# Aqasch/TensorRL-QAS

Hardware: AMD Instinct MI355X
Metric: VQE env-steps/sec (higher is better)
Workload: dtype f64

## Files before the change

tensorrl-qas_amd/csrc/vqe_device.h:

```cpp
#pragma once
#include <hip/hip_runtime.h>
#include <stdint.h>
#ifdef VQE_STAMPS
__device__ unsigned long long g_cby_dbg[8];
__device__ unsigned long long g_cby_in_out[2];
__device__ long long g_cby_t0_unused;
#if defined(__HIP_DEVICE_COMPILE__)
#define CBY_STAMP_RESET() long long cby_t0_ = (long long)__builtin_readcyclecounter(); (void)cby_t0_
#define CBY_STAMP(k)                                                                               \
  {                                                                                                \
    const long long t_ = (long long)__builtin_readcyclecounter();                                  \
    if (ctx.tid == 0 && Ctx::nth > 1) __hip_atomic_fetch_add(&g_cby_dbg[k], (unsigned long long)(t_ - cby_t0_), __ATOMIC_RELAXED, __HIP_MEMORY_SCOPE_AGENT); \
    cby_t0_ = (long long)__builtin_readcyclecounter();                                             \
  }
#else
#define CBY_STAMP_RESET()
#define CBY_STAMP(k)
#endif
#endif
#include "cobyla_m0.h"
#include "vqe_geo.h"

namespace vqe {

// ... 431 lines not shown
    const GateRec* g = staged ? gl : gsrc;
    uint32_t* xm = L.xm;
    uint32_t* zm = L.zm;
    for (int q = 0; q < n; ++q) { xm[q] = 1u << q; zm[q] = 1u << q; }
    uint32_t c = 0;
    int phase = 0, nops = 0;
    auto slot = [&](int q) {
      if (nops < A.max_ops) L.ops[nops] = Op{0u, zm[q], -1, OP_NOP};
      ++nops;
    };
    for (int i = 0; i < G; ++i) {
      if (i >= skip && i < skip_end) continue;
      const GateRec r = g[i];
      if (slots && (r.kind == G_DEPOL1 || r.kind == G_DEPOL2)) {
        slot(r.q0);
        if (r.kind == G_DEPOL2) slot(r.q1);
        continue;
      }
      switch (r.kind) {
        case G_CNOT:
          zm[r.q1] ^= zm[r.q0];
          xm[r.q0] ^= xm[r.q1];
          if ((c >> r.q0) & 1u) c ^= 1u << r.q1;
          break;
        case G_RX: case G_RY: case G_RZ:
          if (nops < A.max_ops)
            L.ops[nops] = Op{xm[r.q0], zm[r.q0], r.pidx, r.kind | (int)(((c >> r.q0) & 1u) << 8)};
          ++nops;
          break;
        case G_RXX: case G_RYY: case G_RZZ:
          if (nops < A.max_ops)
            L.ops[nops] = Op{xm[r.q0] ^ xm[r.q1], zm[r.q0] ^ zm[r.q1], r.pidx,
                             rot2_op(r.kind) | (int)((((c >> r.q0) ^ (c >> r.q1)) & 1u) << 8)};
          ++nops;
          break;
        default: break;
      }
    }
    int permuted = (c != 0);
    for (int q = 0; q < n; ++q) if (xm[q] != (1u << q)) permuted = 1;
    L.meta[0] = nops < A.max_ops ? nops : A.max_ops;
    L.meta[1] = (int32_t)c;
    L.meta[2] = phase;
    L.meta[3] = permuted;
    L.meta[6] = permuted;
    L.meta[7] = (int32_t)c;
  }
  __syncthreads();
}

template <int N>
__device__ __forceinline__ void patch_noise_wave(const BatchArgs& A, int b, uint64_t eval_id, const Lds& L, int skip,
                                                 bool canonical, int lane, int skip_end) {
  const int G = A.gate_count[b];
  const int4* gsrc = (const int4*)(A.gates + A.gate_begin[b]);
  {
    Op* exe = N >= 10 ? L.sched : L.ops;
    const int kmax = L.meta[0];
    const uint64_t lt_mask = lane ? (~0ull >> (64 - lane)) : 0ull;
    const uint64_t nkey = noise_key(A.noise.seed, (uint64_t)b, eval_id);
    uint32_t c = 0;
    int ny = 0, kbase = 0;
    int4 rnext = lane < G ? gsrc[lane] : make_int4(-1, 0, 0, 0);
    for (int base = 0; base < G; base += 64) {
      const int i = base + lane;
      int kind = -1, q0 = 0, q1 = 0, code = 0;
      const int4 r = rnext;
      if (i + 64 < G) rnext = gsrc[i + 64];
      if (i < G && !(i >= skip && i < skip_end)) {
        kind = r.x; q0 = r.y; q1 = r.z < 0 ? 0 : r.z;
        if (kind == G_DEPOL1 || kind == G_DEPOL2) {
          const double u = noise_uniform_k(nkey, (uint64_t)(i - ((skip >= 0 && i >= skip_end) ? skip_end - skip : 0)));
          if (kind == G_DEPOL1) { if (u < A.noise.p1) code = 1 + (int)(u / A.noise.p1 * 3.0); }
          else if (u < A.noise.p2) code = 1 + (int)(u / A.noise.p2 * 15.0);
        }
      }
      const int pa = kind == G_DEPOL1 ? code : (kind == G_DEPOL2 ? (code & 3) : 0);
      const int pb = kind == G_DEPOL2 ? (code >> 2) : 0;
      const uint32_t flip_a = (pa == 1 || pa == 2) ? 1u << q0 : 0u;
      const uint32_t flip_b = (pb == 1 || pb == 2) ? 1u << q1 : 0u;
      const uint32_t cnot_m = kind == G_CNOT ? 1u << q1 : 0u;
      const int nrec = ((kind >= G_RX && kind <= G_DEPOL1) || gate_is_rot2(kind)) ? 1 : (kind == G_DEPOL2 ? 2 : 0);
      const uint32_t w1 = flip_a | ((uint32_t)q0 << 16) | ((uint32_t)q1 << 24) | (gate_is_rot2(kind) ? 1u << 31 : 0u);
      const uint32_t w2 = cnot_m | (flip_b << 16);
      const uint64_t has1 = __ballot(nrec >= 1), has2 = __ballot(nrec == 2);
      const int k0 = kbase + __popcll(has1 & lt_mask) + __popcll(has2 & lt_mask);
      kbase += __popcll(has1) + __popcll(has2);
      ny += __popcll(__ballot(pa == 2)) + __popcll(__ballot(pb == 2));
      uint64_t inv0 = 0, inv1 = 0;
      const int cnt = G - base < 64 ? G - base : 64;
      int j0 = 0;
      if (c == 0) {
        const uint64_t flips = __ballot((flip_a | flip_b) != 0u);
        j0 = flips ? __ffsll((long long)flips) - 1 : cnt;
      }
      for (int j = j0; j < cnt; ++j) {
        const uint32_t a = (uint32_t)__builtin_amdgcn_readlane((int)w1, j);
        const uint32_t bw = (uint32_t)__builtin_amdgcn_readlane((int)w2, j);
        c ^= a & 0xffffu;
        const uint32_t b0 = ((c >> ((a >> 16) & 31u)) ^ ((c >> ((a >> 24) & 31u)) & (a >> 31))) & 1u;
        c ^= (0u - b0) & (bw & 0xffffu);
        inv0 |= (uint64_t)b0 << j;
        c ^= bw >> 16;
        inv1 |= (uint64_t)((c >> ((a >> 24) & 31u)) & 1u) << j;
      }
      auto apply = [&](int pk, int sign, int pauli) {
        if (pk < kmax) {
          Op* o = exe + L.sidx[pk];
          int kd = o->kind;
          if (pauli >= 0) kd = (kd & ~0xff) | ((pauli == 2 || pauli == 3) ? OP_PZ : OP_NOP);
          o->kind = (kd & ~0x100) | (sign << 8);
        }
      };
      if (nrec >= 1) apply(k0, (int)((inv0 >> lane) & 1ull), gate_is_rot(kind) ? -1 : pa);
      if (nrec == 2) apply(k0 + 1, (int)((inv1 >> lane) & 1ull), pb);
    }
    {
      const int ns = N >= 10 ? L.meta[4] : kmax;
      int lead = 0;
      for (int base = ((ns - 1) / 64) * 64; base >= 0; base -= 64) {
        const int k = base + lane;
        const int kd = k < ns ? exe[k].kind : 0;
        const bool nop = k < ns && (kd & 0xff) == OP_NOP;
        const uint64_t m = __ballot(nop);
        const uint64_t behind = lane < 63 ? (m >> (lane + 1)) : 0ull;
        const int in_chunk = 63 - lane;
        int run = behind == ~0ull >> (lane + 1) && lane < 63 ? in_chunk : (lane < 63 ? __ffsll((long long)~behind) - 1 : 0);
        if (run >= in_chunk) run = in_chunk + lead;
        if (k < ns) exe[k].kind = (kd & 0x00ffffff) | ((run < 255 ? run : 255) << 24);
        lead = (m == ~0ull) ? 64 + lead : __ffsll((long long)~m) - 1;
      }
    }
    if (lane == 0) {
      uint32_t cs = c;
      if (N >= 10 && canonical) {
        cs = 0;
        for (int q = 0; q < N; ++q) cs |= (uint32_t)parity32(A.ham.mrow[q] & c) << q;
      }
      L.meta[1] = (int32_t)cs;
      L.meta[2] = (3 * ny) & 3;
      L.meta[3] = L.meta[6] | (c != 0);
      L.meta[7] = (int32_t)c;
    }
  }
}

template <int N>
__device__ __forceinline__ void patch_noise(const BatchArgs& A, int b, uint64_t eval_id, const Lds& L, int skip,
                                            bool canonical, int skip_end = 0) {
  if (threadIdx.x < 64) patch_noise_wave<N>(A, b, eval_id, L, skip, canonical, (int)threadIdx.x, skip_end);
  __syncthreads();
}

}
#include "vqe_reg.h"
namespace vqe {

template <int N>
__device__ __forceinline__ void compile_all(const BatchArgs& A, int b, uint64_t eval_id, const Lds& L, int skip = -1,
                                            bool canonical = true, bool slots = false, int skip_end = 0) {
  compile_ops(A, b, eval_id, L, skip, slots, skip_end);
  if constexpr (N < 10) {
    if (slots) {
      for (int k = threadIdx.x; k < L.meta[0]; k += (int)blockDim.x) L.sidx[k] = (uint16_t)k;
      __syncthreads();
    }
  }
  if constexpr (N >= kRegMinQubits) {
    if (threadIdx.x == 0) schedule_ops<N>(L);
    __syncthreads();
    if (canonical) {
      uint32_t zrow = 0, cbit = 0;
      if (threadIdx.x < N) {
        const uint32_t m = A.ham.mrow[threadIdx.x];
        for (int q = 0; q < N; ++q) if ((m >> q) & 1u) zrow ^= L.zm[q];
        cbit = (uint32_t)parity32(m & (uint32_t)L.meta[1]) << threadIdx.x;
      }
      uint32_t cnew = cbit;
#pragma unroll
      for (int o = 8; o > 0; o >>= 1) cnew |= __shfl_xor(cnew, o, 16);
      __syncthreads();
      if (threadIdx.x < N) L.zm[threadIdx.x] = zrow;
      if (threadIdx.x == 0) L.meta[1] = (int32_t)cnew;
      __syncthreads();
    }
  }
}

template <int N, bool SLOTS = true>
__device__ __forceinline__ void run_ops(const Lds& L, const double* theta, int P, int p_hole = -1) {
  constexpr int kThreads = Geo<N>::NT;
  constexpr uint32_t DIM = 1u << N;
  constexpr int NP = (DIM / 2 + kThreads - 1) / kThreads;
  constexpr int NA = (DIM + kThreads - 1) / kThreads;
  const int tid = threadIdx.x;
  for (int j = tid; j < P; j += kThreads) {
    if (j == p_hole) continue;
    double s, c;
    sincos(0.5 * theta[j - (p_hole >= 0 && j > p_hole)], &s, &c);
    L.cs[j] = make_double2(c, s);
  }
  __syncthreads();
  const int nops = L.meta[0];
  for (int o = 0; o < nops; ++o) {
    const Op op = L.ops[o];
    const int kind = op.kind & 0xff;
    if constexpr (SLOTS) o += (int)((uint32_t)op.kind >> 24);
    if (kind == OP_NOP) continue;
    const int inv = (op.kind >> 8) & 1;
    if (op_is_pair(kind)) {
      const double2 cs = L.cs[op.pidx];
      const int hb = 31 - __clz((int)op.xm);
      if (kind == OP_RX) {
#pragma unroll
        for (int k = 0; k < NP; ++k) {
          const uint32_t q = tid + k * kThreads;
          if (DIM / 2 >= kThreads || q < DIM / 2) {
            const uint32_t p0 = insert0(q, hb), p1 = p0 ^ op.xm;
            const double2 a0 = L.psi[p0], a1 = L.psi[p1];
            L.psi[p0] = make_double2(cs.x * a0.x - cs.y * a1.y, cs.x * a0.y + cs.y * a1.x);
            L.psi[p1] = make_double2(cs.x * a1.x - cs.y * a0.y, cs.x * a1.y + cs.y * a0.x);
          }
        }
      } else if (kind == OP_RY) {
#pragma unroll
        for (int k = 0; k < NP; ++k) {
          const uint32_t q = tid + k * kThreads;
          if (DIM / 2 >= kThreads || q < DIM / 2) {
            const uint32_t p0 = insert0(q, hb), p1 = p0 ^ op.xm;
            const double s0 = (parity32(p0 & op.zm) ^ inv) ? -cs.y : cs.y;
            const double2 a0 = L.psi[p0], a1 = L.psi[p1];
            L.psi[p0] = make_double2(cs.x * a0.x + s0 * a1.x, cs.x * a0.y + s0 * a1.y);
            L.psi[p1] = make_double2(cs.x * a1.x - s0 * a0.x, cs.x * a1.y - s0 * a0.y);
          }
        }
      } else {
#pragma unroll
        for (int k = 0; k < NP; ++k) {
          const uint32_t q = tid + k * kThreads;
          if (DIM / 2 >= kThreads || q < DIM / 2) {
            const uint32_t p0 = insert0(q, hb), p1 = p0 ^ op.xm;
            const double s0 = (parity32(p0 & op.zm) ^ inv) ? cs.y : -cs.y;
            const double2 a0 = L.psi[p0], a1 = L.psi[p1];
            L.psi[p0] = make_double2(cs.x * a0.x - s0 * a1.y, cs.x * a0.y + s0 * a1.x);
            L.psi[p1] = make_double2(cs.x * a1.x - s0 * a0.y, cs.x * a1.y + s0 * a0.x);
          }
        }
      }
    } else if (kind == OP_RZ) {
      const double2 cs = L.cs[op.pidx];
#pragma unroll
      for (int k = 0; k < NA; ++k) {
        const uint32_t p = tid + k * kThreads;
        if (DIM >= kThreads || p < DIM) {
          const double s = (parity32(p & op.zm) ^ inv) ? -cs.y : cs.y;
          const double2 a = L.psi[p];
          L.psi[p] = make_double2(cs.x * a.x - s * a.y, cs.x * a.y + s * a.x);
        }
      }
    } else if (kind == OP_PZ) {
#pragma unroll
      for (int k = 0; k < NA; ++k) {
        const uint32_t p = tid + k * kThreads;
        if ((DIM >= kThreads || p < DIM) && (parity32(p & op.zm) ^ inv)) {
          const double2 a = L.psi[p];
          L.psi[p] = make_double2(-a.x, -a.y);
        }
      }
    }
    __syncthreads();
  }
  if (L.meta[3]) {
    const uint32_t c = (uint32_t)L.meta[1];
    double2 tmp[NA];
#pragma unroll
    for (int k = 0; k < NA; ++k) {
      const uint32_t i = tid + k * kThreads;
      if (DIM >= kThreads || i < DIM) {
        uint32_t v = i ^ c, p = 0;
#pragma unroll
        for (int q = 0; q < N; ++q) p ^= ((v >> q) & 1u) ? L.xm[q] : 0u;
        tmp[k] = L.psi[p];
      }
    }
    __syncthreads();
#pragma unroll
    for (int k = 0; k < NA; ++k) {
      const uint32_t i = tid + k * kThreads;
      if (DIM >= kThreads || i < DIM) L.psi[i] = tmp[k];
    }
    __syncthreads();
  }
}

template <int N>
__device__ __forceinline__ void load_init(const Lds& L, const double2* init) {
  constexpr int kThreads = Geo<N>::NT;
  constexpr uint32_t DIM = 1u << N;
  constexpr int NA = (DIM + kThreads - 1) / kThreads;
#pragma unroll
  for (int k = 0; k < NA; ++k) {
    const uint32_t p = threadIdx.x + k * kThreads;
    if (DIM >= kThreads || p < DIM) L.psi[p] = init[p];
  }
}


constexpr int kEnergyBatch = 4;

#define VQE_ENERGY_PAIRS(X, HB, DEXPR)                                                             \
  {                                                                                                \
    const uint32_t base = insert0(tid, (HB)) << 4, basex = base ^ ((X) << 4);                     \
    uint32_t kbit[KB > 0 ? KB : 1];                                                                \
    _Pragma("unroll") for (int i = 0; i < KB; ++i)                                                \
      kbit[i] = 16u << (LT + i + ((LT + i) >= (HB) ? 1 : 0));                                     \
    double p0s = 0.0, p1s = 0.0;                                                                   \
    _Pragma("unroll") for (int k0 = 0; k0 < NP; k0 += kEnergyBatch) {                             \
      constexpr int NB = NP < kEnergyBatch ? NP : kEnergyBatch;                                   \
      double2 pa[NB], pb[NB];                                                                      \
      _Pragma("unroll") for (int kk = 0; kk < NB; ++kk) {                                         \
        const int k = k0 + kk;                                                                     \
        uint32_t kc = 0;                                                                           \
        _Pragma("unroll") for (int i = 0; i < KB; ++i) if ((k >> i) & 1) kc ^= kbit[i];           \
        const bool live = FULL || tid + (uint32_t)k * kThreads < DIM / 2;                         \
        pb[kk] = live ? *(const double2*)(psi_b + (base ^ kc)) : make_double2(0.0, 0.0);         \
        pa[kk] = live ? *(const double2*)(psi_b + (basex ^ kc)) : make_double2(0.0, 0.0);        \
      }                                                                                            \
      __builtin_amdgcn_sched_barrier(0);                                                           \
      _Pragma("unroll") for (int kk = 0; kk < NB; ++kk) {                                         \
        const int k = k0 + kk;                                                                     \
        const double v = (pa[kk].x * pb[kk].x + pa[kk].y * pb[kk].y) * (DEXPR);                   \
        if (k & 1) p1s += v; else p0s += v;                                                       \
      }                                                                                            \
    }                                                                                              \
    acc0 += p0s;                                                         \
    acc1 += p1s;                                                                                   \
  }

#define VQE_ENERGY_CONSUME(G, D)                                                                   \
  {                                                                                                \
    const GroupMeta m = L.gm[G];                                                                   \
    const uint32_t x = (uint32_t)__builtin_amdgcn_readfirstlane((int)m.x);                        \
    const int hb = __builtin_amdgcn_readfirstlane(m.hb);                                          \
    VQE_ENERGY_PAIRS(x, hb, D[k])                                                                  \
  }

template <int N>
__device__ __forceinline__ void energy_real_lds(const Lds& L, const double* __restrict__ tables, int g0, int g1,
                                                double& acc0, double& acc1) {
  constexpr int kThreads = Geo<N>::NT;
  constexpr uint32_t DIM = 1u << N;
  constexpr int NP = (DIM / 2 + kThreads - 1) / kThreads;
  constexpr int LT = Geo<N>::LT;
  constexpr int KB = N > LT + 1 ? N - LT - 1 : 0;
// ... 308 lines not shown
    for (int j = 0; j < PD - 1; ++j) {
#pragma unroll
      for (int k = 0; k < NP / 2; ++k) buf[j][k] = buf_load_d2(rt, voff[k], (uint32_t)j * GSTRIDE);
      __builtin_amdgcn_sched_barrier(0);
    }
#pragma unroll
    for (int k = 0; k < NP / 2; ++k) buf[PD - 1][k] = make_double2(0.0, 0.0);
    double2 bA[HP], bB[HP];
    uint2 mh[2];
    uint4 mo[2][2];
    const uint32_t tid16 = stid << 4;
    uint32_t tb;
    int ccls;
#define VQE_R_FETCH(S, GI)                                                                         \
    {                                                                                              \
      const ClsMeta* cm_ = L.cm + ((GI) < ncls ? (GI) : ncls - 1);                                 \
      mh[S] = *(const uint2*)cm_;                                                                  \
      mo[S][0] = *(const uint4*)cm_->off;                                                          \
      if constexpr (NP > 4) mo[S][1] = *(const uint4*)(cm_->off + 4);                             \
    }
#define VQE_R_OFF(S, J) ((J) == 0 ? mo[S][0].x : (J) == 1 ? mo[S][0].y : (J) == 2 ? mo[S][0].z : (J) == 3 ? mo[S][0].w : \
                         (J) == 4 ? mo[S][1].x : (J) == 5 ? mo[S][1].y : (J) == 6 ? mo[S][1].z : mo[S][1].w)
#define VQE_R_LOAD(S, HH, PB)                                                                      \
    _Pragma("unroll") for (int kk = 0; kk < HP; ++kk)                                             \
      PB[kk] = lds_load_d2(psi_l, tb + VQE_R_OFF(S, (HH) * HP + kk));
#define VQE_R_OWN(C, J) own[(((J) >> (C)) << ((C) + 1)) | ((J) & ((1 << (C)) - 1))]
#define VQE_R_DV(D, J) (((J) & 1) ? D[(J) / 2].y : D[(J) / 2].x)
#define VQE_R_COMP_C(C, HH, PB, D)                                                                 \
    if constexpr (HP == 4)                                                                         \
      pair_fma4(acc0, acc1, VQE_R_OWN(C, (HH) * 4), VQE_R_OWN(C, (HH) * 4 + 1), VQE_R_OWN(C, (HH) * 4 + 2),     \
                VQE_R_OWN(C, (HH) * 4 + 3), PB, VQE_R_DV(D, (HH) * 4), VQE_R_DV(D, (HH) * 4 + 1),            \
                VQE_R_DV(D, (HH) * 4 + 2), VQE_R_DV(D, (HH) * 4 + 3));                                       \
    else if constexpr (HP == 2)                                                                    \
      pair_fma2(acc0, acc1, VQE_R_OWN(C, (HH) * 2), VQE_R_OWN(C, (HH) * 2 + 1), PB, VQE_R_DV(D, (HH) * 2),     \
                VQE_R_DV(D, (HH) * 2 + 1));                                                                  \
    else                                                                                           \
      pair_fma1(acc0, VQE_R_OWN(C, (HH)), PB, VQE_R_DV(D, (HH)));
#define VQE_R_BODY(C, JJ)                                                                          \
    {                                                                                              \
      VQE_R_COMP_C(C, 0, bA, buf[JJ])                                                              \
      __builtin_amdgcn_sched_barrier(0);                                                           \
      tb = tid16 ^ mh[((JJ) + 1) & 1].x;                                                           \
      VQE_R_LOAD(((JJ) + 1) & 1, 0, bA)                                                            \
      __builtin_amdgcn_sched_barrier(0);                                                           \
      VQE_R_COMP_C(C, 1, bB, buf[JJ])                                                              \
    }
    VQE_R_FETCH(0, 0)
    VQE_R_FETCH(1, 1)
    tb = tid16 ^ mh[0].x;
    VQE_R_LOAD(0, 0, bA)
    for (int g = 0; g < ncls; g += PD) {
#pragma unroll
      for (int j = 0; j < PD; ++j) {
        {
          const int sl = (j + PD - 1) % PD;
          int gr = (j == 0) ? (g == 0 ? PD - 1 : g - 1 + PD) : g + j - 1 + PD;
          gr = gr < ncls ? gr : ncls - 1;
          const uint32_t soff = (uint32_t)gr * GSTRIDE;
#pragma unroll
          for (int k = 0; k < NP / 2; ++k) buf[sl][k] = buf_load_d2(rt, voff[k], soff);
        }
        ccls = __builtin_amdgcn_readfirstlane((int)mh[j & 1].y);
        VQE_R_LOAD(j & 1, 1, bB)
        VQE_R_FETCH(j & 1, g + j + 2)
        __builtin_amdgcn_sched_barrier(0);
        switch (ccls) {
          case 0: VQE_R_BODY(0, j) break;
          case 1: VQE_R_BODY(1, j) break;
          case 2: if constexpr (R > 2) VQE_R_BODY(2, j) break;
          default: if constexpr (R > 3) VQE_R_BODY(3, j) break;
        }
        __builtin_amdgcn_sched_barrier(0);
      }
    }
#undef VQE_R_FETCH
#undef VQE_R_OFF
#undef VQE_R_LOAD
#undef VQE_R_OWN
#undef VQE_R_DV
#undef VQE_R_COMP_C
#undef VQE_R_BODY
  }
  after_pairs();
  unit_energy<N>(L, H, acc0, acc1);
  const int g1 = g0 + H.n_real;
  energy_real_lds<N>(L, tables, gc, g1, acc0, acc1);
  energy_imag_lds<N>(L, tables, g1, H.n_groups, acc0);
  return block_sum<Geo<N>::NW>(acc0 + acc1, L.red);
}

template <int N, bool SLOTS = false, class Hook = NoHook>
__device__ __forceinline__ double lds_evaluate(const BatchArgs& A, const Lds& L, const double* theta, int P,
                                               int p_hole = -1, Hook after_pairs = Hook(), bool cs_ready = false) {
#ifdef VQE_STAMPS
  const long long t0 = clock64();
#endif
  if constexpr (N >= kRegMinQubits) {
    run_ops_reg<N, SLOTS>(L, A.init, theta, P, p_hole, A.dbg, cs_ready);
  } else {
    load_init<N>(L, A.init);
    __syncthreads();
    run_ops<N, SLOTS>(L, theta, P, p_hole);
  }
#ifdef VQE_STAMPS
  const long long t1 = clock64();
#endif
  double e;
  if constexpr (N >= kRegMinQubits) e = reg_energy<N>(L, A.ham, after_pairs); else e = lds_energy<N>(L, A.ham);
#ifdef VQE_STAMPS
  if (threadIdx.x == 0) {
    atomicAdd(A.dbg + 0, 1ull);
    atomicAdd(A.dbg + 1, (unsigned long long)(t1 - t0));
    atomicAdd(A.dbg + 2, (unsigned long long)(clock64() - t1));
  }
#endif
  return e;
}

struct NoSide { __device__ __forceinline__ void operator()() const {} };

template <int K>
struct KeepRegs {
  double2 v;
  KeepRegs<K - 1> rest;
  template <class F> __device__ __forceinline__ void load(F f, int k = 0) { v = f(k); rest.load(f, k + 1); }
  template <class F> __device__ __forceinline__ void store(F f, int k = 0) const { f(k, v); rest.store(f, k + 1); }
};
template <>
struct KeepRegs<0> {
  template <class F> __device__ __forceinline__ void load(F, int = 0) {}
  template <class F> __device__ __forceinline__ void store(F, int = 0) const {}
};

template <int N, bool WIDE = (N >= 10 && Geo<N>::NT >= 256)>
struct StagedCobyla {
  static constexpr int kThreads = Geo<N>::NT;
  typedef cby::CobylaM0<WaveCtx, false, lds_double> CobL;
  static constexpr bool kBlock = WIDE && Geo<N>::NT >= 256;
  static constexpr bool kRowsG = WIDE && Geo<N>::NT == 64;
  typedef cby::CobylaM0<WaveCtx, false, double> CobG;
  typedef cby::CobylaM0<WaveRowsCtx, false, double> CobR;
  __device__ __forceinline__ bool rows_ctx() const { return kRowsG && n > 32; }
#ifndef VQE_BLOCK_TILE
#define VQE_BLOCK_TILE 1
#endif
  static constexpr bool kBlockTile = VQE_BLOCK_TILE && ((size_t)16 << N) >= (Geo<N>::NT / 64) * kCobTileBytes + 4096;
  typedef cby::CobylaM0<BlockCtx<Geo<N>::NT, kBlockTile>, false, double> CobB;
  double* red;
  bool block;
  double* gmem;
  double* lmem;
  double* tile;
  int* pub;
  int n, words;
  bool staged;
  bool resident;
  int want, nfvals;
#ifndef VQE_STAGE_PREFETCH
#define VQE_STAGE_PREFETCH 1
#endif
#ifndef VQE_LIGHT_OUT
#define VQE_LIGHT_OUT 0
#endif
  static constexpr bool PRE = VQE_STAGE_PREFETCH && N >= 10 && Geo<N>::NT >= 256;
  KeepRegs<PRE ? 6 : 0> pre;
  bool pre_valid;
  __device__ __forceinline__ void init(double* global_scratch, const Lds& L, int n_) {
    pre_valid = false;
    gmem = global_scratch;
    resident = L.cob != nullptr;
    lmem = resident ? L.cob : (double*)L.psi;
    tile = L.tile;
    pub = (int*)(L.red + 8);
    n = n_;
    words = (int)cby::scratch_doubles(n, WaveCtx::kPad);
    red = L.red;
    block = kBlock && n > 64;
    staged = resident || (!block && (size_t)words * 8 <= ((size_t)16 << N));
    if (block) words = (int)cby::scratch_doubles(n, CobB::P);
    if (!staged && !block) {
      const int pad = rows_ctx() ? CobR::P : CobG::P;
      words = (int)cby::scratch_doubles_ld(n, pad, cby::lead_dim_global(cby::padded(n, pad)));
    }
  }
  __device__ __forceinline__ double* x() const { return resident ? lmem : gmem; }
  __device__ __forceinline__ const double* state() const { return (resident ? lmem : gmem) + words - cby::kStateDoubles; }
  static constexpr int kStage = 6;
  __device__ __forceinline__ void prefetch() {
    if constexpr (PRE) {
      if (!staged || resident) return;
      const double2* s = (const double2*)gmem;
      const int nw = (words + 1) / 2;
      pre.load([&](int k) {
        const int i = (int)threadIdx.x + k * kThreads;
        return s[i < nw ? i : nw - 1];
      });
      pre_valid = true;
    }
  }
  __device__ __forceinline__ void in() {
    if (!staged || resident) return;
    const double2* s = (const double2*)gmem;
    double2* d = (double2*)lmem;
    const int nw = (words + 1) / 2;
    int first = threadIdx.x;
    if constexpr (PRE) {
      if (pre_valid) {
        pre.store([&](int k, const double2& v) {
          const int i = (int)threadIdx.x + k * kThreads;
          if (i < nw) d[i] = v;
        });
        pre_valid = false;
        first += kStage * kThreads;
      }
    }
    for (int i0 = first; i0 < nw; i0 += kStage * kThreads) {
      double2 v[kStage];
#pragma unroll
      for (int k = 0; k < kStage; ++k) {
        const int i = i0 + k * kThreads;
        v[k] = s[i < nw ? i : nw - 1];
      }
#pragma unroll
      for (int k = 0; k < kStage; ++k) asm volatile("" : "+v"(v[k].x), "+v"(v[k].y));
#pragma unroll
      for (int k = 0; k < kStage; ++k) {
        const int i = i0 + k * kThreads;
        if (i < nw) d[i] = v[k];
      }
    }
    __syncthreads();
  }
  __device__ __forceinline__ bool out(bool full = true, double2* cs_out = nullptr, int P = 0, int p_hole = -1) {
    if (threadIdx.x == 0) { pub[0] = want; pub[1] = nfvals; }
    __syncthreads();
    want = pub[0]; nfvals = pub[1];
    if (!staged || resident) return false;
    const bool light = VQE_LIGHT_OUT && !full && want && cs_out != nullptr;
    if (light) {
      for (int j = threadIdx.x; j < P; j += kThreads) {
        if (j == p_hole) continue;
        double sn, cn;
        sincos(0.5 * lmem[j - (p_hole >= 0 && j > p_hole)], &sn, &cn);
        cs_out[j] = make_double2(cn, sn);
      }
    }
    const double2* s = (const double2*)lmem;
    double2* d = (double2*)gmem;
    const int nw = (words + 1) / 2;
    for (int i0 = threadIdx.x; i0 < nw; i0 += kStage * kThreads) {
      double2 v[kStage];
#pragma unroll
      for (int k = 0; k < kStage; ++k) {
        const int i = i0 + k * kThreads;
        v[k] = s[i < nw ? i : nw - 1];
      }
#pragma unroll
      for (int k = 0; k < kStage; ++k) asm volatile("" : "+v"(v[k].x), "+v"(v[k].y));
#pragma unroll
      for (int k = 0; k < kStage; ++k) {
        const int i = i0 + k * kThreads;
        if (i < nw) d[i] = v[k];
      }
    }
    if (light) {
      asm volatile("s_waitcnt lgkmcnt(0)\n\ts_barrier" ::: "memory");
      return true;
    }
    __syncthreads();
    return false;
  }
  template <bool FIRST, class Cob, class Ptr>
  __device__ __forceinline__ void call(Ptr mem, double f, double rhobeg, double rhoend, int maxfun) {
    Cob cob;
    cob.ctx.tid = Cob::P == 0 ? 0 : (int)(threadIdx.x % (unsigned)decltype(cob.ctx)::nth);
    if constexpr (!std::is_base_of<WaveCtx, decltype(cob.ctx)>::value) cob.ctx.red = red;
    if constexpr (decltype(cob.ctx)::kTile) {
      if constexpr (std::is_base_of<WaveCtx, decltype(cob.ctx)>::value) {
        cob.ctx.tile = (lds_double*)tile;
        cob.ctx.shared = (lds_double*)tile + Cob::kTileDoubles;
      } else {
        cob.ctx.tile = (lds_double*)lmem + (threadIdx.x >> 6) * Cob::kTileDoubles;
        cob.ctx.shared = (lds_double*)lmem + (kThreads / 64) * Cob::kTileDoubles;
      }
    }
    int nn = n;
    if constexpr (N >= 10) asm volatile("" : "+s"(mem), "+s"(nn));
    cob.bind(mem, nn);
    if (FIRST) {
      want = cob.start(rhobeg, rhoend, maxfun);
    } else {
      cob.load_state();
      want = cob.tell(f);
    }
    nfvals = cob.nfvals;
    cob.save_state();
  }
  bool cs_ready;
  template <bool FIRST, class Side>
  __device__ __forceinline__ int run(double f, double rhobeg, double rhoend, int maxfun, Side side, bool full = true,
                                     double2* cs_out = nullptr, int P = 0, int p_hole = -1) {
#ifdef VQE_STAMPS
    const long long t0 = clock64();
#endif
    in();
#ifdef VQE_STAMPS
    const long long t1 = clock64();
#endif
    if (kBlock && block) {
      if constexpr (kBlock) {
        if (kThreads == 64 || (threadIdx.x >= 64 && threadIdx.x < 128)) side();
        call<FIRST, CobB>(gmem, f, rhobeg, rhoend, maxfun);
      }
    } else if (threadIdx.x < 64) {
      if (staged) call<FIRST, CobL>((lds_double*)lmem, f, rhobeg, rhoend, maxfun);
      else if (rows_ctx()) {
        if constexpr (kRowsG) call<FIRST, CobR>(gmem, f, rhobeg, rhoend, maxfun);
      } else call<FIRST, CobG>(gmem, f, rhobeg, rhoend, maxfun);
      if constexpr (kThreads == 64) side();
    } else if (threadIdx.x < 128) {
#ifdef VQE_STAMPS
      const long long ts0 = clock64();
#endif
      side();
#ifdef VQE_STAMPS
      if (threadIdx.x == 64 && !FIRST) atomicAdd(&g_cby_dbg[6], (unsigned long long)(clock64() - ts0));
#endif
    }
#ifdef VQE_STAMPS
    const long long t2 = clock64();
#endif
    cs_ready = out(full, cs_out, P, p_hole);
#ifdef VQE_STAMPS
    if (threadIdx.x == 0 && !FIRST) {
      atomicAdd(&g_cby_dbg[7], (unsigned long long)(t2 - t1));
      atomicAdd(&g_cby_in_out[0], (unsigned long long)(t1 - t0));
      atomicAdd(&g_cby_in_out[1], (unsigned long long)(clock64() - t2));
    }
#endif
    return want;
  }
  __device__ __forceinline__ int start(double rhobeg, double rhoend, int maxfun, bool full = true, double2* cs_out = nullptr,
                                       int P = 0, int p_hole = -1) {
    return run<true>(0.0, rhobeg, rhoend, maxfun, NoSide(), full, cs_out, P, p_hole);
  }
  template <class Side>
  __device__ __forceinline__ int tell(double f, unsigned long long* __restrict__ dbg, Side side, bool full = true,
                                      double2* cs_out = nullptr, int P = 0, int p_hole = -1) {
#ifdef VQE_STAMPS
    const long long t0 = clock64();
#endif
    const int w = run<false>(f, 0.0, 0.0, 0, side, full, cs_out, P, p_hole);
#ifdef VQE_STAMPS
    if (threadIdx.x == 0) atomicAdd(dbg + 4, (unsigned long long)(clock64() - t0));
#endif
    return w;
  }
};

template <int N>
__global__ void __launch_bounds__(Geo<N>::NT) k_lds_energy(BatchArgs A) {
  extern __shared__ __attribute__((aligned(16))) unsigned char smem[];
  const Lds L = carve(smem, N, A.max_ops, A.max_params, A.ham.n_groups, A.max_pair);
  const int b = blockIdx.x;
  const bool noisy = (A.noise.p1 > 0.0 || A.noise.p2 > 0.0);
  stage_groups(A.ham, L);
  if constexpr (N >= 10) stage_cls<N>(A.ham, L);
  compile_all<N>(A, b, 0, L, -1, true, noisy);
  if (noisy) patch_noise<N>(A, b, A.noise.eval_base, L, -1, true);
  double e = lds_evaluate<N, true>(A, L, A.theta + A.par_begin[b], A.par_count[b]);
  if (A.noise.shot_sigma != 0.0) e += A.noise.shot_sigma * noise_gauss(A.noise.seed, (uint64_t)b, A.noise.eval_base);
  if (threadIdx.x == 0) { A.fout[b] = e; if (A.nfev) A.nfev[b] = 1; }
}

template <int N>
__global__ void __launch_bounds__(Geo<N>::NT) k_lds_state(BatchArgs A) {
  constexpr int kThreads = Geo<N>::NT;
  extern __shared__ __attribute__((aligned(16))) unsigned char smem[];
  const Lds L = carve(smem, N, A.max_ops, A.max_params, A.ham.n_groups, A.max_pair);
  const bool noisy_state = (A.noise.p1 > 0.0 || A.noise.p2 > 0.0);
  compile_all<N>(A, 0, 0, L, -1, false, noisy_state);
  if (noisy_state) patch_noise<N>(A, 0, A.noise.eval_base, L, -1, false);
  if constexpr (N >= kRegMinQubits) {
    run_ops_reg<N, true>(L, A.init, A.theta + A.par_begin[0], A.par_count[0]);
  } else {
    load_init<N>(L, A.init);
    __syncthreads();
    run_ops<N>(L, A.theta + A.par_begin[0], A.par_count[0]);
  }
  const int ph = L.meta[2];
  for (uint32_t p = threadIdx.x; p < (1u << N); p += kThreads) {
    double2 a = L.psi[p];
    if (ph == 1) a = make_double2(-a.y, a.x);
    else if (ph == 2) a = make_double2(-a.x, -a.y);
    else if (ph == 3) a = make_double2(a.y, -a.x);
    A.state_out[p] = a;
  }
}

template <int N, bool WIDE = (N >= 10 && Geo<N>::NT >= 256), bool NOISY = false>
__global__ void __launch_bounds__(Geo<N>::NT, Geo<N>::WPS) k_lds_minimize(BatchArgs A) {
  constexpr int kThreads = Geo<N>::NT;
  extern __shared__ __attribute__((aligned(16))) unsigned char smem[];
  const Lds L = carve(smem, N, A.max_ops, A.max_params, A.ham.n_groups, A.max_pair);
  const int b = A.order[blockIdx.x];
  const int P = A.par_count[b];
  const double* theta = A.theta + A.par_begin[b];
  double* xout = A.xout + A.par_begin[b];
  constexpr bool noisy = NOISY;
  const int skip = A.new_gate ? A.new_gate[b] : -1;
  int p_hole = -1;
  int skip_end = skip + 1;
  if (skip >= 0) {
    const GateRec r = A.gates[A.gate_begin[b] + skip];
    if (gate_is_rot(r.kind)) p_hole = r.pidx;
    if (skip + 1 < A.gate_count[b]) {
      const GateRec f = A.gates[A.gate_begin[b] + skip + 1];
      if ((f.kind == G_DEPOL1 && r.kind >= G_RX && r.kind <= G_RZ && f.q0 == r.q0) ||
          (f.kind == G_DEPOL2 && r.kind == G_CNOT && f.q0 == r.q0 && f.q1 == r.q1))
        skip_end = skip + 2;
    }
  }
  const int Popt = P - (p_hole >= 0);
  stage_groups(A.ham, L);
  if constexpr (N >= 10) stage_cls<N>(A.ham, L);
  StagedCobyla<N, WIDE> sc;
  sc.cs_ready = false;
  const bool full_out = N < 10 || A.trace != nullptr;
  int phase = 0, nfev = 1;
  bool need_compile = true;
  bool patched = false;
  double fret = 0.0, flast = 0.0;
  if (Popt > 0) {
    sc.init(A.scratch + A.scratch_begin[b], L, Popt);
    for (int j = threadIdx.x; j < P; j += kThreads)
      if (j != p_hole) sc.x()[j - (p_hole >= 0 && j > p_hole)] = theta[j];
    __syncthreads();
    sc.start(A.rhobeg, A.rhoend, A.maxfun, full_out, L.cs, P, p_hole);
    phase = 1;
  }
  for (;;) {
    const double* th = phase == 0 ? theta : (phase == 1 ? sc.x() : xout);
    const int sk = phase == 2 ? -1 : skip;
    const int ske = phase == 2 ? 0 : skip_end;
    const int ph = phase == 2 ? -1 : p_hole;
    const uint64_t eid = A.noise.eval_base +
                         (phase == 1 ? (uint64_t)sc.nfvals : (phase == 2 ? (uint64_t)A.maxfun + 1 : 0));
    if (need_compile) { compile_all<N>(A, b, 0, L, sk, true, noisy, ske); need_compile = false; patched = false; }
    if (noisy && !patched) patch_noise<N>(A, b, eid, L, sk, true, ske);
    patched = false;
    const bool csr = phase == 1 && sc.cs_ready;
    double e = lds_evaluate<N, NOISY>(A, L, th, P, ph, [&]() { if (phase == 1) sc.prefetch(); }, csr);
    if (A.noise.shot_sigma != 0.0) e += A.noise.shot_sigma * noise_gauss(A.noise.seed, (uint64_t)b, eid);
    bool finished_opt = false;
    if (phase == 0) {
      fret = e;
      for (int j = threadIdx.x; j < P; j += kThreads) {
        xout[j] = A.env_step ? (double)(float)theta[j] : theta[j];
        A.xraw[A.par_begin[b] + j] = theta[j];
      }
      finished_opt = true;
    } else if (phase == 1) {
      flast = e;
      if (A.trace) {
        double* tr = A.trace + ((size_t)b * A.maxfun + (size_t)(sc.nfvals - 1)) * (size_t)(1 + A.max_params);
        if (threadIdx.x == 0) tr[0] = e;
        for (int j = threadIdx.x; j < Popt; j += kThreads) tr[1 + j] = sc.x()[j];
      }
#ifdef VQE_STAMPS
      const long long tt0 = clock64();
#endif
      const uint64_t eid_next = A.noise.eval_base + (uint64_t)sc.nfvals + 1;
      const int want = sc.tell(e, A.dbg, [&]() {
        if (noisy) patch_noise_wave<N>(A, b, eid_next, L, sk, true, (int)(threadIdx.x & 63), ske);
      }, full_out, L.cs, P, p_hole);
      patched = noisy && want;
#ifdef VQE_STAMPS
      if (threadIdx.x == 0) atomicAdd(A.dbg + 3, (unsigned long long)(clock64() - tt0));
#endif
      if (!want) {
        for (int j = threadIdx.x; j < P; j += kThreads) {
          const double v = (j == p_hole) ? theta[j] : sc.x()[j - (p_hole >= 0 && j > p_hole)];
          xout[j] = A.env_step ? (double)(float)v : v;
          A.xraw[A.par_begin[b] + j] = v;
        }
        const double* st = sc.state();
        fret = ((int)st[11] == cby::DONE_RHOEND && (int)st[10] == 1) ? flast : st[4];
        nfev = sc.nfvals;
        finished_opt = true;
      }
    } else {
      fret = e;
      break;
    }
    if (finished_opt) {
      if (!A.env_step) break;
      __syncthreads();
      phase = 2;
      need_compile = true;
    }
  }
  if (threadIdx.x == 0) { A.fout[b] = fret; A.nfev[b] = nfev; }
}

}
```

tensorrl-qas_amd/csrc/vqe_reg.h:

```cpp
#pragma once
#include "vqe_geo.h"

namespace vqe {

enum : int { OP_RELAYOUT = 5 };

struct LayoutRec {
  uint32_t e[5];
  uint32_t pos;
  uint32_t pos8;
  uint32_t pad;
};

struct Basis {
  uint32_t* e;
  int32_t* piv;
  int k;
  __device__ void clear() { k = 0; }
  __device__ uint32_t reduce(uint32_t v) const {
    for (int i = 0; i < k; ++i) if ((v >> piv[i]) & 1u) v ^= e[i];
    return v;
  }
  __device__ bool add(uint32_t v) {
    v = reduce(v);
// ... 34 lines not shown
  for (int i = 0; i < R; ++i) if ((svec >> i) & 1u) w ^= pat[i];
  return w;
}

template <int N>
__device__ __forceinline__ void schedule_ops(const Lds& L) {
  constexpr int R = N - Geo<N>::LT;
  const int nraw = L.meta[0];
  int ns = 0, nl = 0;
  Basis B;
  B.e = (uint32_t*)L.sb;
  B.piv = (int32_t*)L.sb + 8;
  auto open_layout = [&](int from) {
    B.clear();
    for (int k = from; k < nraw && B.k < R; ++k) {
      const int kd = L.ops[k].kind & 0xff;
      if (op_is_pair(kd)) B.add(L.ops[k].xm);
    }
    for (int b = N - 1; b >= 0 && B.k < R; --b) B.add(1u << b);
    emit_layout<N>(B, &L.lay[nl]);
    ++nl;
  };
  open_layout(0);
  for (int o = 0; o < nraw; ++o) {
    const Op op = L.ops[o];
    const int kd = op.kind & 0xff;
    uint32_t j = 0;
    if (op_is_pair(kd)) {
      if (B.reduce(op.xm) != 0) {
        open_layout(o);
        L.sched[ns++] = Op{(uint32_t)(nl - 1), 0u, -1, OP_RELAYOUT};
      }
      j = B.coords(op.xm);
    }
    uint32_t svec = 0;
    for (int i = 0; i < R; ++i) svec |= (uint32_t)parity32(op.zm & B.e[i]) << i;
    L.sidx[o] = (uint16_t)ns;
    L.sched[ns++] = Op{sign_word<R>(svec), op.zm, op.pidx >= 0 ? op.pidx * 16 : 0, op.kind | (int32_t)(j << 16)};
  }
  L.sched[ns] = Op{0u, 0u, 0, 0};
  L.meta[4] = ns;
  L.meta[5] = nl;
}

template <int LT>
__device__ __forceinline__ uint32_t deposit(uint32_t tid, uint32_t pos, uint32_t pos8) {
  uint32_t b = 0;
#pragma unroll
  for (int j = 0; j < 8; ++j) b |= ((tid >> j) & 1u) << ((pos >> (4 * j)) & 15u);
  if (LT > 8) b |= ((tid >> 8) & 1u) << pos8;
  return b;
}

template <int R>
__device__ __forceinline__ uint32_t combo(const uint32_t (&e)[5], int r) {
  uint32_t v = 0;
#pragma unroll
  for (int i = 0; i < R; ++i) if ((r >> i) & 1) v ^= e[i];
  return v;
}

__device__ __forceinline__ double flip_if(double v, uint32_t w, int r) {
  const uint32_t hi = (uint32_t)__double2hiint(v) ^ (((w >> r) & 1u) << 31);
  return __hiloint2double((int)hi, __double2loint(v));
}

__device__ __forceinline__ void rot2x2(double& x0, double& y0, double& x1, double& y1, double c, double s0,
                                       double s1) {
  double t0, t1;
  asm("v_mul_f64 %4, %7, %1\n\t"
      "v_mul_f64 %5, %8, %3\n\t"
      "v_mul_f64 %1, %6, %1\n\t"
      "v_mul_f64 %3, %6, %3\n\t"
      "v_fmac_f64 %1, %7, %0\n\t"
      "v_fmac_f64 %3, %8, %2\n\t"
      "v_fma_f64 %0, %6, %0, -%4\n\t"
      "v_fma_f64 %2, %6, %2, -%5"
      : "+v"(x0), "+v"(y0), "+v"(x1), "+v"(y1), "=&v"(t0), "=&v"(t1)
      : "v"(c), "v"(s0), "v"(s1));
}

template <int NA, int J>
__device__ __forceinline__ void rx_pairs(double2 (&amp)[NA], double c, double s) {
  static_assert(J > 0 && J < NA, "partner mask out of range");
  constexpr int HB = 31 - __builtin_clz(J);
#pragma unroll
  for (int r = 0; r < NA; ++r) {
    if ((r >> HB) & 1) continue;
    const int r2 = r ^ J;
    rot2x2(amp[r].x, amp[r2].y, amp[r2].x, amp[r].y, c, s, s);
  }
}

template <int NA, int J>
__device__ __forceinline__ void ry_pairs(double2 (&amp)[NA], double c, double s, uint32_t w) {
  constexpr int HB = 31 - __builtin_clz(J);
#pragma unroll
  for (int r = 0; r < NA; ++r) {
    if ((r >> HB) & 1) continue;
    const int r2 = r ^ J;
    const double s0 = flip_if(s, w, r);
    rot2x2(amp[r2].x, amp[r].x, amp[r2].y, amp[r].y, c, s0, s0);
  }
}

template <int NA, int J>
__device__ __forceinline__ void ryy_pairs(double2 (&amp)[NA], double c, double s, uint32_t nw) {
  constexpr int HB = 31 - __builtin_clz(J);
#pragma unroll
  for (int r = 0; r < NA; ++r) {
    if ((r >> HB) & 1) continue;
    const int r2 = r ^ J;
    const double s0 = flip_if(s, nw, r);
    rot2x2(amp[r].x, amp[r2].y, amp[r2].x, amp[r].y, c, s0, s0);
  }
}

#define VQE_PAIR_CASE(J, CALL) case J: if constexpr (J < NA) { CALL; } break;
#define VQE_PAIR_SWITCH(j, F, ...)                                                                 \
  switch (j) {                                                                                     \
    VQE_PAIR_CASE(1, (F<NA, 1>(__VA_ARGS__))) VQE_PAIR_CASE(2, (F<NA, 2>(__VA_ARGS__)))            \
    VQE_PAIR_CASE(3, (F<NA, 3>(__VA_ARGS__))) VQE_PAIR_CASE(4, (F<NA, 4>(__VA_ARGS__)))            \
    VQE_PAIR_CASE(5, (F<NA, 5>(__VA_ARGS__))) VQE_PAIR_CASE(6, (F<NA, 6>(__VA_ARGS__)))            \
    VQE_PAIR_CASE(7, (F<NA, 7>(__VA_ARGS__))) VQE_PAIR_CASE(8, (F<NA, 8>(__VA_ARGS__)))            \
    VQE_PAIR_CASE(9, (F<NA, 9>(__VA_ARGS__))) VQE_PAIR_CASE(10, (F<NA, 10>(__VA_ARGS__)))          \
    VQE_PAIR_CASE(11, (F<NA, 11>(__VA_ARGS__))) VQE_PAIR_CASE(12, (F<NA, 12>(__VA_ARGS__)))        \
    VQE_PAIR_CASE(13, (F<NA, 13>(__VA_ARGS__))) VQE_PAIR_CASE(14, (F<NA, 14>(__VA_ARGS__)))        \
    VQE_PAIR_CASE(15, (F<NA, 15>(__VA_ARGS__))) VQE_PAIR_CASE(16, (F<NA, 16>(__VA_ARGS__)))        \
    VQE_PAIR_CASE(17, (F<NA, 17>(__VA_ARGS__))) VQE_PAIR_CASE(18, (F<NA, 18>(__VA_ARGS__)))        \
    VQE_PAIR_CASE(19, (F<NA, 19>(__VA_ARGS__))) VQE_PAIR_CASE(20, (F<NA, 20>(__VA_ARGS__)))        \
    VQE_PAIR_CASE(21, (F<NA, 21>(__VA_ARGS__))) VQE_PAIR_CASE(22, (F<NA, 22>(__VA_ARGS__)))        \
    VQE_PAIR_CASE(23, (F<NA, 23>(__VA_ARGS__))) VQE_PAIR_CASE(24, (F<NA, 24>(__VA_ARGS__)))        \
    VQE_PAIR_CASE(25, (F<NA, 25>(__VA_ARGS__))) VQE_PAIR_CASE(26, (F<NA, 26>(__VA_ARGS__)))        \
    VQE_PAIR_CASE(27, (F<NA, 27>(__VA_ARGS__))) VQE_PAIR_CASE(28, (F<NA, 28>(__VA_ARGS__)))        \
    VQE_PAIR_CASE(29, (F<NA, 29>(__VA_ARGS__))) VQE_PAIR_CASE(30, (F<NA, 30>(__VA_ARGS__)))        \
    VQE_PAIR_CASE(31, (F<NA, 31>(__VA_ARGS__)))                                                    \
    default: break;                                                                                \
  }

template <int N, bool SLOTS = false>
__device__ __forceinline__ void run_ops_reg(const Lds& L, const double2* __restrict__ init, const double* theta, int P,
                                   int p_hole = -1, unsigned long long* __restrict__ dbg = nullptr, bool cs_ready = false) {
#ifdef VQE_STAMPS
  const long long ts0 = clock64();
  long long trel = 0;
#endif
  constexpr int kThreads = Geo<N>::NT;
  constexpr int LT = Geo<N>::LT;
  constexpr int R = N - LT;
  constexpr int NA = 1 << R;
  int tid = threadIdx.x;
  asm volatile("" : "+v"(tid));
  if (!cs_ready) {
    for (int j = tid; j < P; j += kThreads) {
      if (j == p_hole) continue;
      double s, c;
      sincos(0.5 * theta[j - (p_hole >= 0 && j > p_hole)], &s, &c);
      L.cs[j] = make_double2(c, s);
    }
  }
  double2 amp[NA];
  uint32_t e[5];
  typedef __attribute__((address_space(3))) unsigned char lds_byte;
  lds_byte* psi_l = (lds_byte*)L.psi;
  auto lds_get = [&](uint32_t off) {
    const d2v_t v = *(const __attribute__((address_space(3))) d2v_t*)(psi_l + off);
    return make_double2(v.x, v.y);
  };
  auto lds_put = [&](uint32_t off, const double2& a) {
    d2v_t v; v.x = a.x; v.y = a.y;
    *(__attribute__((address_space(3))) d2v_t*)(psi_l + off) = v;
  };
  uint32_t base = deposit<LT>(tid, L.lay[0].pos, L.lay[0].pos8);
  {
    const LayoutRec lr = L.lay[0];
#pragma unroll
    for (int i = 0; i < 5; ++i) e[i] = lr.e[i] << 4;
    const unsigned char* init_b = (const unsigned char*)init;
#pragma unroll
    for (int r = 0; r < NA; ++r) amp[r] = *(const double2*)(init_b + ((base << 4) ^ combo<R>(e, r)));
  }
  __builtin_amdgcn_s_waitcnt(0x0F70);
  __syncthreads();
  const int nops = L.meta[4];
#ifdef VQE_STAMPS
  const long long ts1 = clock64();
#endif
  const unsigned char* cs_b = (const unsigned char*)L.cs;
  Op nxt = L.sched[0];
  double2 ncs = *(const double2*)(cs_b + nxt.pidx);
  for (int o = 0; o < nops; ++o) {
    const Op op = nxt;
    const double2 cs = ncs;
    if constexpr (SLOTS) o += (int)((uint32_t)__builtin_amdgcn_readfirstlane(op.kind) >> 24);
    nxt = L.sched[o + 1];
    ncs = *(const double2*)(cs_b + nxt.pidx);
    const int kind = op.kind & 0xff;
    if (kind == OP_RELAYOUT) {
#ifdef VQE_STAMPS
      const long long tr0 = clock64();
#endif
      __syncthreads();
      {
        const uint32_t b16 = base << 4;
#pragma unroll
        for (int r = 0; r < NA; ++r) lds_put(b16 ^ combo<R>(e, r), amp[r]);
      }
      const LayoutRec lr = L.lay[op.xm];
#pragma unroll
      for (int i = 0; i < 5; ++i) e[i] = lr.e[i] << 4;
      base = deposit<LT>(tid, lr.pos, lr.pos8);
      __syncthreads();
      {
        const uint32_t b16 = base << 4;
#pragma unroll
        for (int r = 0; r < NA; ++r) amp[r] = lds_get(b16 ^ combo<R>(e, r));
      }
#ifdef VQE_STAMPS
      trel += clock64() - tr0;
#endif
      continue;
    }
    if (kind == OP_NOP) continue;
    const int inv = (op.kind >> 8) & 1;
    const uint32_t flip = (uint32_t)(parity32(op.zm & base) ^ inv);
    const uint32_t w = op.xm ^ (0u - flip);
    const int jm = (op.kind >> 16) & 0xff;
    if (kind == OP_RX) {
      VQE_PAIR_SWITCH(jm, rx_pairs, amp, cs.x, cs.y)
    } else if (kind == OP_RY) {
      VQE_PAIR_SWITCH(jm, ry_pairs, amp, cs.x, cs.y, w)
    } else if (kind == OP_RZ) {
#pragma unroll
      for (int r = 0; r < NA; r += 2)
        rot2x2(amp[r].x, amp[r].y, amp[r + 1].x, amp[r + 1].y, cs.x, flip_if(cs.y, w, r), flip_if(cs.y, w, r + 1));
    } else if (kind == OP_PZ) {
#pragma unroll
      for (int r = 0; r < NA; ++r) amp[r] = make_double2(flip_if(amp[r].x, w, r), flip_if(amp[r].y, w, r));
    } else if (kind == OP_RYY) {
      VQE_PAIR_SWITCH(jm, ryy_pairs, amp, cs.x, cs.y, ~w)
    }
  }
#ifdef VQE_STAMPS
  const long long ts2 = clock64();
#endif
  uint32_t ib = (uint32_t)L.meta[1] << 4;
  uint32_t ae[5] = {0u, 0u, 0u, 0u, 0u};
#pragma unroll
  for (int q = 0; q < N; ++q) {
    const uint32_t z = L.zm[q];
    ib ^= (uint32_t)parity32(z & base) << (q + 4);
#pragma unroll
    for (int i = 0; i < R; ++i) ae[i] |= (uint32_t)parity32(z & (e[i] >> 4)) << (q + 4);
  }
  __syncthreads();
#pragma unroll
  for (int r = 0; r < NA; ++r) lds_put(ib ^ combo<R>(ae, r), amp[r]);
  __syncthreads();
#ifdef VQE_STAMPS
  if (threadIdx.x == 0 && dbg) {
    atomicAdd(dbg + 5, (unsigned long long)(ts1 - ts0));
    atomicAdd(dbg + 6, (unsigned long long)trel);
    atomicAdd(dbg + 7, (unsigned long long)(clock64() - ts2));
  }
#endif
}

}
```

Baseline: 13330.

## Rotate COBYLA owner wave and spread per-parameter work across waves

Adds a helper that, when the parameter count fits in the block, assigns each parameter to a thread spaced out by a stride so the work lands on different wavefronts instead of all on wave 0. It also rotates which wave runs the serial COBYLA step (and which runs the side task) based on the function-evaluation count, so the serial optimizer work no longer always lands on wave 0. The aim is to balance per-wave load and reduce stalls on a single SIMD. Risks include extra index arithmetic, changed state ownership across waves, and LDS or register state that may assume wave 0.

```diff
diff --git a/tensorrl-qas_amd/csrc/vqe_device.h b/tensorrl-qas_amd/csrc/vqe_device.h
--- a/tensorrl-qas_amd/csrc/vqe_device.h
+++ b/tensorrl-qas_amd/csrc/vqe_device.h
@@ -607,6 +607,21 @@
   __syncthreads();
 }
 
+#ifndef VQE_SERIAL_WAVE0
+#define VQE_SERIAL_WAVE0 0
+#endif
+template <int NT, class F>
+__device__ __forceinline__ void for_each_param(int P, int tid, F f) {
+  if ((VQE_SERIAL_WAVE0 & 2) || P > NT) {
+    for (int j = tid; j < P; j += NT) f(j);
+    return;
+  }
+  constexpr int LT = 31 - __builtin_clz((unsigned)NT);
+  const int sh = P > 1 ? LT - (32 - __builtin_clz((unsigned)(P - 1))) : LT;
+  const int j = tid >> sh;
+  if ((j << sh) == tid && j < P) f(j);
+}
+
 }
 #include "vqe_reg.h"
 namespace vqe {
@@ -649,12 +664,12 @@
   constexpr int NP = (DIM / 2 + kThreads - 1) / kThreads;
   constexpr int NA = (DIM + kThreads - 1) / kThreads;
   const int tid = threadIdx.x;
-  for (int j = tid; j < P; j += kThreads) {
-    if (j == p_hole) continue;
+  for_each_param<kThreads>(P, tid, [&](int j) {
+    if (j == p_hole) return;
     double s, c;
     sincos(0.5 * theta[j - (p_hole >= 0 && j > p_hole)], &s, &c);
     L.cs[j] = make_double2(c, s);
-  }
+  });
   __syncthreads();
   const int nops = L.meta[0];
   for (int o = 0; o < nops; ++o) {
@@ -1269,6 +1284,7 @@
   double* lmem;
   double* tile;
   int* pub;
+  int owner;
   int n, words;
   bool staged;
   bool resident;
@@ -1349,18 +1365,18 @@
     __syncthreads();
   }
   __device__ __forceinline__ bool out(bool full = true, double2* cs_out = nullptr, int P = 0, int p_hole = -1) {
-    if (threadIdx.x == 0) { pub[0] = want; pub[1] = nfvals; }
+    if ((int)threadIdx.x == owner * 64) { pub[0] = want; pub[1] = nfvals; }
     __syncthreads();
     want = pub[0]; nfvals = pub[1];
     if (!staged || resident) return false;
     const bool light = VQE_LIGHT_OUT && !full && want && cs_out != nullptr;
     if (light) {
-      for (int j = threadIdx.x; j < P; j += kThreads) {
-        if (j == p_hole) continue;
+      for_each_param<kThreads>(P, (int)threadIdx.x, [&](int j) {
+        if (j == p_hole) return;
         double sn, cn;
         sincos(0.5 * lmem[j - (p_hole >= 0 && j > p_hole)], &sn, &cn);
         cs_out[j] = make_double2(cn, sn);
-      }
+      });
     }
     const double2* s = (const double2*)lmem;
     double2* d = (double2*)gmem;
@@ -1424,24 +1440,28 @@
 #ifdef VQE_STAMPS
     const long long t1 = clock64();
 #endif
+    constexpr int kWaves = kThreads / 64;
+    const int wave = (int)(threadIdx.x >> 6);
+    owner = (FIRST || kWaves == 1 || (VQE_SERIAL_WAVE0 & 1) || (kBlock && block))
+                ? 0 : (__builtin_amdgcn_readfirstlane(nfvals) & (kWaves - 1));
     if (kBlock && block) {
       if constexpr (kBlock) {
         if (kThreads == 64 || (threadIdx.x >= 64 && threadIdx.x < 128)) side();
         call<FIRST, CobB>(gmem, f, rhobeg, rhoend, maxfun);
       }
-    } else if (threadIdx.x < 64) {
+    } else if (wave == owner) {
       if (staged) call<FIRST, CobL>((lds_double*)lmem, f, rhobeg, rhoend, maxfun);
       else if (rows_ctx()) {
         if constexpr (kRowsG) call<FIRST, CobR>(gmem, f, rhobeg, rhoend, maxfun);
       } else call<FIRST, CobG>(gmem, f, rhobeg, rhoend, maxfun);
       if constexpr (kThreads == 64) side();
-    } else if (threadIdx.x < 128) {
+    } else if (wave == ((owner + 1) & (kWaves - 1))) {
 #ifdef VQE_STAMPS
       const long long ts0 = clock64();
 #endif
       side();
 #ifdef VQE_STAMPS
-      if (threadIdx.x == 64 && !FIRST) atomicAdd(&g_cby_dbg[6], (unsigned long long)(clock64() - ts0));
+      if ((threadIdx.x & 63) == 0 && !FIRST) atomicAdd(&g_cby_dbg[6], (unsigned long long)(clock64() - ts0));
 #endif
     }
 #ifdef VQE_STAMPS
@@ -1449,7 +1469,7 @@
 #endif
     cs_ready = out(full, cs_out, P, p_hole);
 #ifdef VQE_STAMPS
-    if (threadIdx.x == 0 && !FIRST) {
+    if ((int)threadIdx.x == owner * 64 && !FIRST) {
       atomicAdd(&g_cby_dbg[7], (unsigned long long)(t2 - t1));
       atomicAdd(&g_cby_in_out[0], (unsigned long long)(t1 - t0));
       atomicAdd(&g_cby_in_out[1], (unsigned long long)(clock64() - t2));
@@ -1550,8 +1570,9 @@
   double fret = 0.0, flast = 0.0;
   if (Popt > 0) {
     sc.init(A.scratch + A.scratch_begin[b], L, Popt);
-    for (int j = threadIdx.x; j < P; j += kThreads)
+    for_each_param<kThreads>(P, (int)threadIdx.x, [&](int j) {
       if (j != p_hole) sc.x()[j - (p_hole >= 0 && j > p_hole)] = theta[j];
+    });
     __syncthreads();
     sc.start(A.rhobeg, A.rhoend, A.maxfun, full_out, L.cs, P, p_hole);
     phase = 1;
@@ -1572,10 +1593,10 @@
     bool finished_opt = false;
     if (phase == 0) {
       fret = e;
-      for (int j = threadIdx.x; j < P; j += kThreads) {
+      for_each_param<kThreads>(P, (int)threadIdx.x, [&](int j) {
         xout[j] = A.env_step ? (double)(float)theta[j] : theta[j];
         A.xraw[A.par_begin[b] + j] = theta[j];
-      }
+      });
       finished_opt = true;
     } else if (phase == 1) {
       flast = e;
@@ -1596,11 +1617,11 @@
       if (threadIdx.x == 0) atomicAdd(A.dbg + 3, (unsigned long long)(clock64() - tt0));
 #endif
       if (!want) {
-        for (int j = threadIdx.x; j < P; j += kThreads) {
+        for_each_param<kThreads>(P, (int)threadIdx.x, [&](int j) {
           const double v = (j == p_hole) ? theta[j] : sc.x()[j - (p_hole >= 0 && j > p_hole)];
           xout[j] = A.env_step ? (double)(float)v : v;
           A.xraw[A.par_begin[b] + j] = v;
-        }
+        });
         const double* st = sc.state();
         fret = ((int)st[11] == cby::DONE_RHOEND && (int)st[10] == 1) ? flast : st[4];
         nfev = sc.nfvals;
diff --git a/tensorrl-qas_amd/csrc/vqe_reg.h b/tensorrl-qas_amd/csrc/vqe_reg.h
--- a/tensorrl-qas_amd/csrc/vqe_reg.h
+++ b/tensorrl-qas_amd/csrc/vqe_reg.h
@@ -210,12 +210,12 @@
   int tid = threadIdx.x;
   asm volatile("" : "+v"(tid));
   if (!cs_ready) {
-    for (int j = tid; j < P; j += kThreads) {
-      if (j == p_hole) continue;
+    for_each_param<kThreads>(P, tid, [&](int j) {
+      if (j == p_hole) return;
       double s, c;
       sincos(0.5 * theta[j - (p_hole >= 0 && j > p_hole)], &s, &c);
       L.cs[j] = make_double2(c, s);
-    }
+    });
   }
   double2 amp[NA];
   uint32_t e[5];
```

Measured after the change: 12750. 4.4% lower.
